# usnistgov/object-detection-yolov3

Measured on AMD Instinct MI355X. Metric: images/sec (train fwd+bwd) bs=8 416x416, higher is better.
Workload: dtype f32

## Files before the change

include/yolo3hip.h:

```cpp
#ifndef YOLO3HIP_H
#define YOLO3HIP_H

#include <math.h>
#include <stddef.h>
#include <stdint.h>

#ifdef __cplusplus
extern "C" {
#endif

#define Y3_OK 0
#define Y3_EINVAL (-1)
#define Y3_ELAUNCH (-2)

typedef void* y3_stream_t;

const char* y3_last_error(void);
int y3_debug_div(int x, int d);
int y3_version(void);

#define Y3_EPI_LRELU 1u
#define Y3_EPI_ACCUM 2u
#define Y3_CONV_X3 4u
int y3_x3_split_weights(const float* w, void* planes, int taps, int rows, int k_per_row, y3_stream_t stream);
int y3_x3_split_weights_batched(const float* arena, void* planes_arena, const int* table_dev, int nlayers, int total_blocks, y3_stream_t stream);
int y3_x3_prepare_weights_batched(const float* params, float* params_t, void* planes, void* planes_t, const int* table_dev, int nlayers,
                                  int total_tiles, y3_stream_t stream);

typedef struct y3_tensor {
    float* ptr;
    int n, h, w, c;
    int ld;
} y3_tensor;

int y3_conv2d_fwd(const y3_tensor* src, const float* wt, const float* bias, int ksize, int stride,
                  const y3_tensor* dst, unsigned flags, float alpha,
                  const float* scale, const float* shift, const y3_tensor* resid,
                  float* stats, void* workspace, size_t workspace_bytes, y3_stream_t stream);
int y3_conv2d_stats_tiles(int m, int cin, int ksize, int cout);
size_t y3_conv2d_fwd_workspace(int m, int cin, int ksize, int cout);
int y3_conv2d_stats_tiles_x(int m, int cin, int ksize, int cout, unsigned flags);
size_t y3_conv2d_fwd_workspace_x(int m, int cin, int ksize, int cout, unsigned flags);
int y3_conv2d_x3_ok(int m, int c, int ntaps, int nout);
int y3_conv2d_dgrad_x3_ok(const y3_tensor* ddst, int ksize, int stride, const y3_tensor* dsrc);
size_t y3_conv2d_plan(int m, int cin, int ksize, int cout, int* out13);
size_t y3_conv2d_plan_x(int m, int cin, int ksize, int cout, unsigned flags, int* out13);

int y3_conv2d_dgrad(const y3_tensor* ddst, const float* wt_t, int ksize, int stride,
                    const y3_tensor* dsrc, unsigned flags, void* workspace, size_t workspace_bytes,
                    y3_stream_t stream);
size_t y3_conv2d_dgrad_workspace(const y3_tensor* ddst, int ksize, int stride, const y3_tensor* dsrc);
size_t y3_conv2d_dgrad_workspace_x(const y3_tensor* ddst, int ksize, int stride, const y3_tensor* dsrc, unsigned flags);
int y3_conv2d_dgrad_bn(const y3_tensor* ddst, const float* wt_t, int ksize, int stride, const y3_tensor* dsrc,
                       unsigned flags, const y3_tensor* bn_a, float* bn_partials,
                       void* workspace, size_t workspace_bytes, y3_stream_t stream);
int y3_conv2d_dgrad_bn_tiles(const y3_tensor* ddst, int ksize, int stride, const y3_tensor* dsrc);
int y3_conv2d_dgrad_bn_tiles_x(const y3_tensor* ddst, int ksize, int stride, const y3_tensor* dsrc, unsigned flags);
size_t y3_conv2d_dgrad_plan_x(const y3_tensor* ddst, int ksize, int stride, const y3_tensor* dsrc, unsigned flags, int* out51);

int y3_conv2d_wgrad(const y3_tensor* src, const y3_tensor* ddst, int ksize, int stride,
                    float* dw, void* workspace, size_t workspace_bytes, y3_stream_t stream);
size_t y3_conv2d_wgrad_workspace(const y3_tensor* src, const y3_tensor* ddst, int ksize, int stride);
int y3_conv2d_wgrad_x(const y3_tensor* src, const y3_tensor* ddst, int ksize, int stride,
                      float* dw, unsigned flags, void* workspace, size_t workspace_bytes, y3_stream_t stream);
size_t y3_conv2d_wgrad_workspace_x(const y3_tensor* src, const y3_tensor* ddst, int ksize, int stride, unsigned flags);
int y3_conv2d_wgrad_x3_ok(int m, int cin, int ksize, int cout);
size_t y3_conv2d_wgrad_plan(int m, int cin, int ksize, int cout, int* out8);
size_t y3_conv2d_wgrad_plan_x(int m, int cin, int ksize, int cout, unsigned flags, int* out8);

int y3_transpose_weights(const float* wt, float* wt_t, int taps, int cin, int cout, y3_stream_t stream);
int y3_transpose_weights_batched(const float* params, float* params_t, const int* table_dev, int nlayers,
                                 int total_tiles, y3_stream_t stream);

int y3_bn_stats_finalize(const float* stats, int tiles, int c, int count,
                         const float* gamma, const float* beta, float eps, float momentum,
                         float* moving_mean, float* moving_var,
                         float* save_mean, float* save_rstd, float* scale, float* shift,
                         y3_stream_t stream);
int y3_bn_fold_inference(const float* gamma, const float* beta, const float* moving_mean,
                         const float* moving_var, float eps, int c, float* scale, float* shift,
                         y3_stream_t stream);
int y3_bn_fold_inference_batched(const float* params, const float* moving, float* chan, const int* table_dev,
                                 int nlayers, float eps, y3_stream_t stream);
int y3_bn_apply(const y3_tensor* a, const float* scale, const float* shift, const y3_tensor* resid,
                const y3_tensor* y, y3_stream_t stream);
int y3_bn_bwd_stats(const y3_tensor* dy, const y3_tensor* a, const y3_tensor* dres, int dres_accumulate,
                    const float* gamma, const float* save_mean, const float* save_rstd, float alpha,
                    float* dgamma, float* dbeta, float* dbias, float* coef,
                    void* workspace, size_t workspace_bytes, y3_stream_t stream);
size_t y3_bn_bwd_workspace(int m, int c);
int y3_bn_bwd_apply(const y3_tensor* dy, const y3_tensor* a, const float* coef, float alpha,
                    const y3_tensor* dz, y3_stream_t stream);
int y3_bn_bwd_apply_fanin(const y3_tensor* dy, const y3_tensor* a, const float* coef, float alpha,
                          const y3_tensor* dz, const y3_tensor* dres, int dres_accumulate, y3_stream_t stream);
int y3_bn_bwd_finalize_tiles(const float* partials, int tiles, int c, int count, const float* gamma,
                             const float* save_mean, const float* save_rstd, float alpha,
                             float* dgamma, float* dbeta, float* dbias, float* coef, y3_stream_t stream);
int y3_bn_frozen_bwd(const y3_tensor* dy, const y3_tensor* a, const y3_tensor* dres, int dres_accumulate,
                     const float* scale, const float* moving_mean, const float* moving_var, float eps, float alpha,
                     const y3_tensor* dz, float* dgamma, float* dbeta, float* dbias,
                     void* workspace, size_t workspace_bytes, y3_stream_t stream);
size_t y3_bn_frozen_bwd_workspace(int m, int c);

int y3_upsample_sum2x_fwd(const y3_tensor* in, const y3_tensor* out, y3_stream_t stream);
int y3_upsample_sum2x_bwd(const y3_tensor* dout, const y3_tensor* din, y3_stream_t stream);

#define Y3_SPP_MAX_PLANE 4096
int y3_spp_fwd(const y3_tensor* src, const y3_tensor* dst, y3_stream_t stream);
int y3_spp_fwd_bf16(const y3_tensor* src, const y3_tensor* dst, y3_stream_t stream);
int y3_spp_bwd(const y3_tensor* src, const y3_tensor* ddst, const y3_tensor* dsrc, int accumulate, y3_stream_t stream);

#define Y3_BF16_NO_PATCH 8u
int y3_conv2d_fwd_bf16(const y3_tensor* src, const void* wt_t_bf16, const float* bias, int ksize, int stride,
                       const y3_tensor* dst, int dst_is_f32, unsigned flags, float alpha,
                       const float* scale, const float* shift, const y3_tensor* resid, y3_stream_t stream);
size_t y3_conv2d_fwd_bf16_workspace(int m, int cin, int ksize, int cout);
int y3_conv2d_fwd_bf16_ws(const y3_tensor* src, const void* wt_t_bf16, const float* bias, int ksize, int stride,
                          const y3_tensor* dst, int dst_is_f32, unsigned flags, float alpha,
                          const float* scale, const float* shift, const y3_tensor* resid,
                          void* workspace, size_t workspace_bytes, y3_stream_t stream);
#define Y3_BF16_ROUTE_PP 1
#define Y3_BF16_ROUTE_C32 2
#define Y3_BF16_ROUTE_C64 3
#define Y3_BF16_ROUTE_RING 4
size_t y3_conv2d_fwd_bf16_plan(const y3_tensor* src, const void* wt_t_bf16, const float* bias, int ksize, int stride,
                               const y3_tensor* dst, int dst_is_f32, unsigned flags, float alpha,
// ... 269 lines not shown
```

object-detection-yolov3_amd/csrc/conv.hip:

```cpp
#include <stdlib.h>

#include <type_traits>
#include <utility>

#include "common.h"
#include "conv_plan.h"

template <int BM, int BN, int WM, int WN, int BK>
__global__ __launch_bounds__(64 * WM * WN) void conv_igemm_kernel(const ConvArgs p) {
    constexpr int THREADS = 64 * WM * WN;
    constexpr int LDA = BK + 4;
    constexpr int TM = BM / WM, TN = BN / WN, MB = TM / 32, NB = TN / 32;
    constexpr int KV = BK / 4;
    constexpr int A_TOTAL = BM * KV, A_LOADS = (A_TOTAL + THREADS - 1) / THREADS;
    constexpr int BN4 = BN / 4;
    constexpr int B_TOTAL = BK * BN4, B_LOADS = (B_TOTAL + THREADS - 1) / THREADS;
    static_assert(THREADS % KV == 0 && TM % 32 == 0 && TN % 32 == 0, "tile shape");

    __shared__ __attribute__((aligned(16))) float As[2][BM * LDA];
    __shared__ __attribute__((aligned(16))) float Bs[2][BK * BN];
    __shared__ float red[2][WM][BN];

    const int tid = threadIdx.x, lane = tid & 63, wave = tid >> 6;
    const int l31 = lane & 31, lh = lane >> 5;
// ... 893 lines not shown
    p.bn_part = a.bn_part;
    p.bn_a_ld = a.bn_a_ld;
    p.bn_a_bytes = a.bn_a ? (unsigned)((a.dense_dst ? (long long)a.M : (long long)a.src_n * a.DH * a.DW) * a.bn_a_ld * 4) : 0u;
    p.bn_row0 = 0;
    p.H = a.H;
    p.W = a.W;
    p.logC = a.logC;
    p.cmask = a.cmask;
    p.src_ld = a.src_ld;
    p.OH = a.OH;
    p.OW = a.OW;
    p.sh = a.sh;
    p.sw = a.sw;
    p.DH = a.DH;
    p.DW = a.DW;
    p.dsh = a.dsh;
    p.dsw = a.dsw;
    p.doh = a.doh;
    p.dow = a.dow;
    p.dst_ld = a.dst_ld;
    p.resid_ld = a.resid_ld;
    p.Nout = a.Nout;
    p.K = a.K;
    p.M = a.M;
    p.flags = a.flags;
    p.alpha = a.alpha;
    *f = p;
    return true;
}
static void set_split(FastArgs& f, const ConvPlan& pl) {
    f.dv_s0 = y3_make_div(pl.s0);
    f.dv_s1 = y3_make_div(pl.s1);
    f.sk_f = pl.f;
    f.sk_s0 = pl.s0;
    f.sk_s1 = pl.s1;
    f.sk_n0 = pl.f * pl.s0;
    f.sk_chunk0 = pl.chunk0;
    f.sk_chunk1 = pl.chunk1;
}

static int launch_igemm(const ConvArgs& a, const GemmDesc& d, void* workspace, size_t workspace_bytes, hipStream_t st) {
    ConvArgs p = a;
    const int ntaps = p.K / p.C;
    if (p.x3 && !d.x3) {
        y3_set_error("conv: Y3_CONV_X3 does not take this shape (C %d, Nout %d, K %d): ask y3_conv2d_x3_ok() first", p.C, p.Nout, p.K);
        return Y3_EINVAL;
    }
    ConvPlan pl = d.pl;
    if (no_room(pl.ws_bytes, workspace, workspace_bytes)) whole_tiles(pl, even_steps(p.K / pl.t.bk));
    const TileCfg t = pl.t;
    p.nbn = y3_cdiv(p.Nout, t.bn);
    FastArgs f;
    if (d.fast && make_fast(p, ntaps, t.bk, &f)) {
        f.nbn = p.nbn;
        f.nbm = y3_cdiv(p.M, t.bm);
        f.col_major = ((long long)p.K * p.Nout * 4 > 2048LL * 1024) ? 1 : 0;
        f.nb_fast = f.col_major ? f.nbm : f.nbn;
        f.dv_nb = y3_make_div(f.nb_fast);
        set_split(f, pl);
        f.sk_slab0 = pl.s0 > 1 ? 0 : f.sk_n0;
        f.tickets = pl.ws_bytes ? (int*)workspace : nullptr;
        if (f.tickets)
            if (int e = check_tickets("conv2d", workspace, st)) return e;
        f.slab = pl.ws_bytes ? (float*)((char*)workspace + Y3_WS_HEADER) : nullptr;
        const int grid = f.sk_n0 + (pl.tiles - pl.f) * pl.s1;
        const bool dense = p.dense_dst != 0;
        if (t.bk != 16) {
            y3_set_error("conv: the fast kernel is built for K steps of 16 (tile %dx%dx%d)", t.bm, t.bn, t.bk);
            return Y3_EINVAL;
        }
        if (p.bn_a && !dense) {
            y3_set_error("conv: BatchNorm-backward statistics need the dense fast kernel with K steps of 16");
            return Y3_EINVAL;
        }
        if (d.x3) {
            if (pl.short_last && pl.f == pl.tiles) f.x3_mode |= 8;
            if (!y3_x3_launch(f, t.bm, t.bn, dense, grid, st)) {
                y3_set_error("conv: no x3 kernel for tile %dx%d", t.bm, t.bn);
                return Y3_EINVAL;
            }
            Y3_CHECK_LAUNCH("conv_x3");
            return Y3_OK;
        }
        if (!launch_fast(t, f, dense, grid, st)) {
            y3_set_error("conv: no fast kernel for tile %dx%dx%d", t.bm, t.bn, t.bk);
            return Y3_EINVAL;
        }
        Y3_CHECK_LAUNCH("conv_igemm_fast");
        return Y3_OK;
    }
    if (p.bn_a || d.x3) {
        y3_set_error("conv: %s not available on the generic kernel (shape %d x %d x %d)", d.x3 ? "Y3_CONV_X3 is" : "BatchNorm-backward statistics are", p.M, p.Nout, p.K);
        return Y3_EINVAL;
    }
    if (!launch_generic(t, p, pl.tiles, st)) {
        y3_set_error("conv: no kernel for tile %dx%dx%d", t.bm, t.bn, t.bk);
        return Y3_EINVAL;
    }
    Y3_CHECK_LAUNCH("conv_igemm");
    return Y3_OK;
}

extern "C" int y3_conv2d_fwd(const y3_tensor* src, const float* wt, const float* bias, int ksize, int stride, const y3_tensor* dst,
                             unsigned flags, float alpha, const float* scale, const float* shift, const y3_tensor* resid, float* stats,
                             void* workspace, size_t workspace_bytes, y3_stream_t stream) {
    if (int e = check_tensor(src, "conv2d_fwd src")) return e;
    if (int e = check_tensor(dst, "conv2d_fwd dst")) return e;
    Y3_CHECK_ARG(wt, "conv2d_fwd: null weights");
    Y3_CHECK_ARG(ksize == 1 || ksize == 3, "conv2d_fwd: ksize %d unsupported", ksize);
    Y3_CHECK_ARG(stride == 1 || stride == 2, "conv2d_fwd: stride %d unsupported", stride);
    Y3_CHECK_ARG((src->c & 3) == 0, "conv2d_fwd: Cin=%d must be a multiple of 4", src->c);
    const int OH = (src->h + stride - 1) / stride, OW = (src->w + stride - 1) / stride;
    Y3_CHECK_ARG(dst->n == src->n && dst->h == OH && dst->w == OW, "conv2d_fwd: dst geometry %dx%dx%d != expected %dx%dx%d", dst->n,
                 dst->h, dst->w, src->n, OH, OW);
    Y3_CHECK_ARG((scale == nullptr) == (shift == nullptr), "conv2d_fwd: scale/shift must both be given");
    ConvArgs p = {};
    p.src = src->ptr;
    p.wt = wt;
    p.dst = dst->ptr;
    p.bias = bias;
    p.scale = scale;
    p.shift = shift;
    p.stats = stats;
    if (resid) {
        if (int e = check_tensor(resid, "conv2d_fwd resid")) return e;
        Y3_CHECK_ARG(resid->n == dst->n && resid->h == dst->h && resid->w == dst->w && resid->c == dst->c, "conv2d_fwd: resid geometry");
        p.resid = resid->ptr;
        p.resid_ld = resid->ld;
    }
    const int taps = ksize * ksize;
    if (int e = set_channels(src->c, taps, &p.logC, &p.cmask)) return e;
    const int pbh = y3_same_pad_before(src->h, ksize, stride), pbw = y3_same_pad_before(src->w, ksize, stride);
    for (int kh = 0; kh < ksize; ++kh)
        for (int kw = 0; kw < ksize; ++kw) {
            const int t = kh * ksize + kw;
            const int dh = kh - pbh, dw = kw - pbw;
            Y3_CHECK_ARG(dh >= -1 && dh <= 2 && dw >= -1 && dw <= 2, "conv2d_fwd: tap offset out of range");
            p.tap_dhdw |= (unsigned long long)((dh + 1) | ((dw + 1) << 2)) << (4 * t);
            p.tap_wsel |= (unsigned long long)t << (4 * t);
        }
    p.H = src->h;
    p.W = src->w;
    p.C = src->c;
    p.src_ld = src->ld;
    p.OH = OH;
    p.OW = OW;
    p.sh = p.sw = stride;
    p.DH = OH;
    p.DW = OW;
    p.dsh = p.dsw = 1;
    p.dst_ld = dst->ld;
    p.dense_dst = 1;
    p.Nout = dst->c;
    p.K = taps * src->c;
    p.M = src->n * OH * OW;
    p.flags = flags & ~Y3_CONV_X3;
    p.x3 = (flags & Y3_CONV_X3) ? 1 : 0;
    p.alpha = alpha;
    p.src_n = src->n;
    p.wt_rows = taps * src->c;
    return launch_igemm(p, describe_gemm(p), workspace, workspace_bytes, (hipStream_t)stream);
}

static int launch_dgrad_multi(const ConvArgs* cls, int ncls, MultiPlan pl, void* workspace, size_t workspace_bytes, hipStream_t st) {
    if (no_room(pl.ws, workspace, workspace_bytes)) {
        for (int c = 0; c < ncls; ++c) whole_tiles(pl.c[c], even_steps(cls[c].K / 16));
// ... 204 lines not shown
```

object-detection-yolov3_amd/csrc/conv_fast.h:

```cpp
#pragma once
#include <type_traits>
#include <utility>

#include "common.h"
#include "conv_plan.h"

struct FastArgs {
    const float* src;
    const float* wt;
    int Cper;
    int x3_mode;
    int korder;
    Y3Div dv_taps;
    float* dst;
    const float* bias;
    const float* scale;
    const float* shift;
    const float* resid;
    float* stats;
    int tap_off[9];
    int tap_wrow[9];
    int tg_nx, tg_off0, tg_offy, tg_offx, tg_w0, tg_wy, tg_wx;
    int tg_mul;
    int tap_dh[9], tap_dw[9];
    unsigned src_bytes, wt_bytes, dst_bytes, resid_bytes;
    int ntaps;
    int H, W, logC, cmask, src_ld;
    int OH, OW, sh, sw;
    int DH, DW, dsh, dsw, doh, dow, dst_ld;
    int resid_ld;
    int Nout, K, M;
    unsigned flags;
    float alpha;
    int nbn, nbm, col_major;
    int nb_fast, ohw;
    Y3Div dv_nb, dv_s0, dv_s1, dv_ohw, dv_ow;
    int sk_f, sk_n0, sk_s0, sk_s1, sk_chunk0, sk_chunk1;
    int sk_slab0;
    float* slab;
    int* tickets;
    const float* bn_a;
    float* bn_part;
    unsigned bn_a_bytes;
    int bn_a_ld;
    int bn_row0;
};

#define Y3_OOB 0x80000000u

#ifdef Y3_TIMING
__device__ int y3_abl_dev = 0;
#define Y3_ABL_INIT() const int y3_abl = __builtin_amdgcn_readfirstlane(y3_abl_dev)
#define Y3_ABL(bit) (y3_abl & (bit))
__device__ unsigned long long* y3_timing_buf = nullptr;
#define Y3_TSTAMP(i)                                                                                                    \
    do {                                                                                                                \
        if (y3_timing_buf && threadIdx.x == 0) y3_timing_buf[(size_t)blockIdx.x * 8 + (i)] = __builtin_amdgcn_s_memtime(); \
    } while (0)
#else
#define Y3_TSTAMP(i)
#define Y3_ABL_INIT()
#define Y3_ABL(bit) 0
#endif

template <int... I, class F>
__device__ __forceinline__ void y3_for_each_ic(std::integer_sequence<int, I...>, F&& f) {
    (f(std::integral_constant<int, I>{}), ...);
}
template <int MASK, int N>
__device__ __forceinline__ void y3_sgb() {
    if constexpr (N > 0) __builtin_amdgcn_sched_group_barrier(MASK, N, 0);
}
template <int COUNT, int MASK, int MFMAS = 1>
__device__ __forceinline__ void y3_sgb_pairs() {
    if constexpr (COUNT > 0) {
        y3_sgb<0x008, MFMAS>();
        y3_sgb<MASK, 1>();
        y3_sgb_pairs<COUNT - 1, MASK, MFMAS>();
    }
}

struct WgradArgs {
    const float* src;
    const float* ddst;
    float* out;
    unsigned long long tap_dhdw;
    int H, W, C, logC, cmask, src_ld;
    int OH, OW, sh, sw;
    int dd_ld, Nout, K, M;
    int chunk;
    int nbn, tiles, splits;
    unsigned src_bytes, dd_bytes;
    int* tickets;
    float* dw;
    int ohw, ntaps;
    Y3Div dv_tiles, dv_nbn, dv_ohw, dv_ow;
};

bool y3_wgrad_x3_launch(const WgradArgs& p, int bkr, int bn, unsigned grid, hipStream_t st);

bool y3_x3_launch(const FastArgs& p, int bm, int bn, bool dense, int grid, hipStream_t st);
struct FastArgs4 {
    FastArgs a[4];
    int first[5];
};
bool y3_x3_multi_launch(const FastArgs4& m, int bn, bool bns, int grid, hipStream_t st);
bool y3_x3_tile_ok(int bm, int bn);

struct FastWork {
    int tid, lane, wave, l31, lh, wm, wn;
    int bid0, bid, kz, nz;
    int bm, bn, m0, n0, kbeg, kend;
    int ohw, OW, aK, aM, aH, aW, src_ld, csh, csw, ntaps, Nout;
    Y3Div dv_ohw, dv_ow;
};

template <int BM, int BN, int WM, int WN, int BK, bool KZMAJOR = false, bool SHORTLAST = false>
__device__ __forceinline__ FastWork conv_fast_decode(const FastArgs& p, const int braw, const int grid) {
    FastWork w;
    const int tid = threadIdx.x, lane = tid & 63, wave = tid >> 6;
    const int l31 = lane & 31, lh = lane >> 5;
    const int wm = wave / WN, wn = wave % WN;
    int sk_n0 = p.sk_n0, sk_s0 = p.sk_s0, sk_s1 = p.sk_s1, sk_f = p.sk_f, sk_c0 = p.sk_chunk0, sk_c1 = p.sk_chunk1;
    int col_major = p.col_major, nb_fast = p.nb_fast, ohw = p.ohw, OW = p.OW, aK = p.K, aM = p.M, aH = p.H, aW = p.W;
    int src_ld = p.src_ld, csh = p.sh, csw = p.sw, ntaps = p.ntaps, Nout = p.Nout;
    unsigned dnb_m = p.dv_nb.mul, ds0_m = p.dv_s0.mul, ds1_m = p.dv_s1.mul, dohw_m = p.dv_ohw.mul, dow_m = p.dv_ow.mul;
    int dnb_s = p.dv_nb.shift, ds0_s = p.dv_s0.shift, ds1_s = p.dv_s1.shift, dohw_s = p.dv_ohw.shift, dow_s = p.dv_ow.shift;
    Y3_PIN_S(sk_n0); Y3_PIN_S(sk_s0); Y3_PIN_S(sk_s1); Y3_PIN_S(sk_f); Y3_PIN_S(sk_c0); Y3_PIN_S(sk_c1);
    Y3_PIN_S(col_major); Y3_PIN_S(nb_fast); Y3_PIN_S(ohw); Y3_PIN_S(OW); Y3_PIN_S(aK); Y3_PIN_S(aM); Y3_PIN_S(aH); Y3_PIN_S(aW);
    Y3_PIN_S(src_ld); Y3_PIN_S(csh); Y3_PIN_S(csw); Y3_PIN_S(ntaps); Y3_PIN_S(Nout);
    Y3_PIN_S(dnb_m); Y3_PIN_S(ds0_m); Y3_PIN_S(ds1_m); Y3_PIN_S(dohw_m); Y3_PIN_S(dow_m);
    Y3_PIN_S(dnb_s); Y3_PIN_S(ds0_s); Y3_PIN_S(ds1_s); Y3_PIN_S(dohw_s); Y3_PIN_S(dow_s);
    const Y3Div dv_nb = {dnb_m, dnb_s}, dv_s0 = {ds0_m, ds0_s}, dv_s1 = {ds1_m, ds1_s}, dv_ohw = {dohw_m, dohw_s}, dv_ow = {dow_m, dow_s};

    int bid0 = braw < sk_n0 ? y3_xcd_remap(braw, sk_n0) : sk_n0 + y3_xcd_remap(braw - sk_n0, grid - sk_n0);
    if (SHORTLAST && (p.x3_mode & 8) && sk_n0 == grid && sk_s0 > 1) {
        const int s = sk_s0, tiles = sk_f, nl = tiles * (s - 1);
        const int x = braw & 7, j = braw >> 3;
        const int ql = nl >> 3, rl = nl & 7;
        const int nlx = ql + (x < rl ? 1 : 0), l0 = x * ql + min(x, rl);
        if (j < nlx) {
            const int a = l0 + j, col = a / (nb_fast * (s - 1)), r = a - col * nb_fast * (s - 1), kzp = r / nb_fast;
            bid0 = (col * nb_fast + (r - kzp * nb_fast)) * s + kzp;
        } else {
            int s0x = 0;
            for (int y = 0; y < x; ++y) s0x += ((grid - y + 7) >> 3) - (ql + (y < rl ? 1 : 0));
            bid0 = (s0x + j - nlx) * s + (s - 1);
        }
    } else if (KZMAJOR && col_major) {
        const bool ra = bid0 < sk_n0;
        const int sl = ra ? sk_s0 : sk_s1;
        if (sl > 1) {
            const int t0 = ra ? 0 : sk_f, t1 = ra ? sk_f : sk_f + y3_div(grid - sk_n0, dv_s1);
            int a = ra ? bid0 : bid0 - sk_n0, base = t0;
            int n = min(t1, (y3_div(t0, dv_nb) + 1) * nb_fast) - t0;
            if (a >= n * sl) {
                a -= n * sl;
                base += n;
                const int col = a / (nb_fast * sl);
                a -= col * nb_fast * sl;
                base += col * nb_fast;
                n = min(nb_fast, t1 - base);
            }
            const int kzp = a / n;
            bid0 = (ra ? 0 : sk_n0) + (base + (a - kzp * n) - t0) * sl + kzp;
        }
    }
    int bid, kz, nz, kchunk;
    if (bid0 < sk_n0) {
        bid = y3_div(bid0, dv_s0);
        kz = bid0 - bid * sk_s0;
        nz = sk_s0;
        kchunk = sk_c0;
    } else {
        const int t = bid0 - sk_n0;
        const int q = y3_div(t, dv_s1);
        bid = sk_f + q;
        kz = t - q * sk_s1;
        nz = sk_s1;
        kchunk = sk_c1;
    }
    const int tq = y3_div(bid, dv_nb), tr = bid - tq * nb_fast;
    const int bm = col_major ? tr : tq;
    const int bn = col_major ? tq : tr;
    const int m0 = bm * BM, n0 = bn * BN;
    const int kbeg = kz * kchunk * BK;
    const int kend = min(aK, kbeg + kchunk * BK);
    w.tid = tid; w.lane = lane; w.wave = wave; w.l31 = l31; w.lh = lh; w.wm = wm; w.wn = wn;
    w.bid0 = bid0; w.bid = bid; w.kz = kz; w.nz = nz;
    w.bm = bm; w.bn = bn; w.m0 = m0; w.n0 = n0; w.kbeg = kbeg; w.kend = kend;
// ... 288 lines not shown
```

object-detection-yolov3_amd/csrc/conv_plan.cpp:

```cpp
#include <stdlib.h>
#include "host.h"
#include "conv_plan.h"

static TileCfg pick_tile(int M, int Nout) {
    TileCfg t;
    if (Nout <= 32)
        t = {128, 32, 16};
    else if (Nout <= 64)
        t = {128, 64, 16};
    else {
        const long long t128 = (long long)y3_cdiv(M, 128) * y3_cdiv(Nout, 128);
        const long long t64x128 = (long long)y3_cdiv(M, 64) * y3_cdiv(Nout, 128);
        if (t128 >= 600)
            t = {128, 128, 16};
        else if (t64x128 >= 600)
            t = {64, 128, 16};
        else
            t = {64, 64, 16};
    }
    return t;
}
void whole_tiles(ConvPlan& pl, int chunk) {
    pl.f = pl.tiles;
    pl.s0 = pl.s1 = 1;
// ... 49 lines not shown
            if (sc > 16) break;
            if ((long long)tiles * sc <= x3_slots)
                c_lo = c;
            else if (c_hi == 0 && (c_lo == 0 || sc > count_for(c_lo)))
                c_hi = c;
        }
        const int s_lo = c_lo > 0 ? count_for(c_lo) : 1;
        if (s_lo > 1) {
            pl.s0 = pl.s1 = s_lo;
            pl.chunk0 = pl.chunk1 = c_lo;
        }
        if (c_hi > 0 && ntaps == 9) {
            const int s_hi = count_for(c_hi), last = nk - (s_hi - 1) * c_hi;
            if ((long long)tiles * s_hi <= x3_slots + x3_slots / 16 && 3 * last <= c_hi) {
                pl.f = tiles;
                pl.s0 = pl.s1 = s_hi;
                pl.chunk0 = pl.chunk1 = c_hi;
                pl.short_last = 1;
                c_hi = 0;
            }
        }
        if (c_hi > 0) {
            const int s_hi = count_for(c_hi);
            const int f = (int)((x3_slots - (long long)tiles * s_lo) / (s_hi - s_lo));
            if (f > 0) {
                pl.f = f < tiles ? f : tiles;
                pl.s0 = s_hi;
                pl.chunk0 = c_hi;
            }
        }
    }
    pl.stats_tiles = y3_cdiv(M, pl.t.bm);
    size_slabs(pl, even_steps(nk));
    return pl;
}
static ConvPlan plan_conv(int M, int Nout, int K, bool fast_ok) {
    ConvPlan pl;
    pl.t = pick_tile(M, Nout);
    const int tiles = y3_cdiv(M, pl.t.bm) * y3_cdiv(Nout, pl.t.bn);
    const int nk = K / pl.t.bk;
    const int whole = nk > 0 ? nk : 1;
    pl.tiles = tiles;
    whole_tiles(pl, whole);
    constexpr int want = 2000;
    constexpr int min_k = 256;
    constexpr int cus = 256;
    constexpr int few_max = 512;
    const bool few_tiles = tiles <= few_max || ((long long)tiles * 2 <= want && K >= 2048);
    if (fast_ok && tiles <= Y3_MAX_TICKETS && few_tiles && K >= 2 * min_k) {
        int ks = (int)((want + tiles / 2) / tiles);
        const int maxs = K / min_k;
        if (ks > maxs) ks = maxs;
        if (ks > 16) ks = 16;
        if (ks > 1) {
            pl.chunk0 = even_steps(y3_cdiv(nk, ks));
            pl.s0 = y3_cdiv(nk, pl.chunk0);
        }
    } else if (fast_ok && tiles <= Y3_MAX_TICKETS && tiles > cus && nk >= 8) {
        const int F = tiles / cus * cus, R = tiles - F;
        if (R > 0) {
            int best = 1;
            double best_cost = 1.0;
            for (int S = 2; S <= 6 && S * 4 <= nk; ++S) {
                const double cost = (double)y3_cdiv((long long)R * S, cus) / S + 0.03 * (S - 1);
                if (cost < best_cost - 1e-9) {
                    best_cost = cost;
                    best = S;
                }
            }
            if (best > 1) {
                pl.f = F;
                pl.chunk1 = even_steps(y3_cdiv(nk, best));
                pl.s1 = y3_cdiv(nk, pl.chunk1);
            }
        }
    }
    pl.stats_tiles = y3_cdiv(M, pl.t.bm);
    size_slabs(pl, whole);
    return pl;
}
static bool fast_shape_ok(int C, int Nout, int K, int ntaps) {
    return !getenv("Y3_NO_FAST") && C % 16 == 0 && K % 16 == 0 && (ntaps == 1 || y3_is_pow2(C));
}
static GemmDesc describe_gemm(int M, int C, int ntaps, int Nout, unsigned flags) {
    GemmDesc d;
    const int K = ntaps * C;
    d.x3 = (flags & Y3_CONV_X3) && x3_shape_ok(C, Nout, K, ntaps);
    d.fast = d.x3 || fast_shape_ok(C, Nout, K, ntaps);
    d.pl = d.x3 ? plan_conv_x3(M, Nout, K, ntaps) : plan_conv(M, Nout, K, d.fast);
    return d;
}

extern "C" int y3_conv2d_x3_ok(int m, int c, int ntaps, int nout) {
    return (m > 0 && (ntaps == 1 || ntaps == 9 || ntaps == 2 || ntaps == 4) && x3_shape_ok(c, nout, ntaps * c, ntaps)) ? 1 : 0;
}
extern "C" int y3_conv2d_stats_tiles_x(int m, int cin, int ksize, int cout, unsigned flags) {
    return describe_gemm(m, cin, ksize * ksize, cout, flags).pl.stats_tiles;
}
extern "C" size_t y3_conv2d_fwd_workspace_x(int m, int cin, int ksize, int cout, unsigned flags) {
    return describe_gemm(m, cin, ksize * ksize, cout, flags).pl.ws_bytes;
}
extern "C" int y3_conv2d_stats_tiles(int m, int cin, int ksize, int cout) { return y3_conv2d_stats_tiles_x(m, cin, ksize, cout, 0u); }
extern "C" size_t y3_conv2d_fwd_workspace(int m, int cin, int ksize, int cout) { return y3_conv2d_fwd_workspace_x(m, cin, ksize, cout, 0u); }

extern "C" size_t y3_conv2d_plan(int m, int cin, int ksize, int cout, int* out13) { return y3_conv2d_plan_x(m, cin, ksize, cout, 0u, out13); }
extern "C" size_t y3_conv2d_plan_x(int m, int cin, int ksize, int cout, unsigned flags, int* out13) {
    const GemmDesc d = describe_gemm(m, cin, ksize * ksize, cout, flags);
    const ConvPlan& pl = d.pl;
    if (out13) {
        const int v[13] = {pl.t.bm, pl.t.bn, pl.t.bk, pl.tiles, pl.f, pl.s0, pl.s1, pl.chunk0, pl.chunk1,
                           pl.f * pl.s0 + (pl.tiles - pl.f) * pl.s1, pl.stats_tiles, (d.fast ? 1 : 0) | (pl.short_last ? 2 : 0), ksize * ksize * cin / pl.t.bk};
        for (int i = 0; i < 13; ++i) out13[i] = v[i];
    }
    return pl.ws_bytes;
}

bool fast_geom(const ConvArgs& a, int ntaps, int bk, FastGeom* g) {
    if (a.C % bk != 0 || a.K % bk != 0) return false;
    if (ntaps > 1 && !y3_is_pow2(a.C)) return false;
    g->min_off = 0;
    for (int t = 0; t < ntaps; ++t) {
        const int code = (int)((a.tap_dhdw >> (4 * t)) & 15ull);
        g->dh[t] = (code & 3) - 1;
        g->dw[t] = (code >> 2) - 1;
        const int off = (g->dh[t] * a.W + g->dw[t]) * a.src_ld;
        if (off < g->min_off) g->min_off = off;
    }
    const long long total = (long long)a.src_n * a.H * a.W * a.src_ld - g->min_off;
    const long long wtotal = (long long)(a.wt_rows) * a.Nout;
    if (total * 4 >= 0x7fffffffLL || wtotal * (a.x3 ? 6 : 4) >= 0x7fffffffLL) return false;
    g->src_bytes = (unsigned)(total * 4);
    g->wt_bytes = (unsigned)(wtotal * (a.x3 ? 6 : 4));
    for (int t = 0; t < ntaps; ++t) {
        g->off[t] = ((g->dh[t] * a.W + g->dw[t]) * a.src_ld - g->min_off) * 4;
        g->wrow[t] = (int)((a.tap_wsel >> (4 * t)) & 15ull) * a.C;
    }
    int nx = 1;
    while (nx < ntaps && g->dh[nx] == g->dh[0]) ++nx;
    if (ntaps % nx != 0 || nx > 3) return false;
    g->nx = nx;
    const int offx = nx > 1 ? g->off[1] - g->off[0] : 0, wx = nx > 1 ? g->wrow[1] - g->wrow[0] : 0;
    const int offy = ntaps > nx ? g->off[nx] - g->off[0] : 0, wy = ntaps > nx ? g->wrow[nx] - g->wrow[0] : 0;
    for (int t = 0; t < ntaps; ++t)
        if (g->off[t] != g->off[0] + (t / nx) * offy + (t % nx) * offx || g->wrow[t] != g->wrow[0] + (t / nx) * wy + (t % nx) * wx)
            return false;
    const long long dpix = a.dense_dst ? (long long)a.M : (long long)a.src_n * a.DH * a.DW;
    const long long db = dpix * a.dst_ld * 4, rb = dpix * (long long)a.resid_ld * 4;
    if (db >= 0x7fffffffLL || rb >= 0x7fffffffLL) return false;
    g->dst_bytes = (unsigned)db;
    g->resid_bytes = (unsigned)rb;
    return true;
}

GemmDesc describe_gemm(const ConvArgs& a) { return describe_gemm(a.M, a.C, a.K / a.C, a.Nout, a.x3 ? Y3_CONV_X3 : 0u); }

int set_channels(int C, int taps, int* logC, int* cmask) {
    if (taps == 1) {
        *logC = 31;
        *cmask = 0x7fffffff;
        return 0;
    }
    Y3_CHECK_ARG(y3_is_pow2(C) && C >= 4, "3x3 conv needs power-of-two channels >= 4 (got %d)", C);
    *logC = y3_ilog2(C);
    *cmask = C - 1;
    return 0;
}

static bool plan_dgrad_multi_f32(const ConvArgs* cls, int ncls, MultiPlan* pl) {
    int mmax = 0;
    for (int c = 0; c < ncls; ++c) mmax = cls[c].M > mmax ? cls[c].M : mmax;
    TileCfg t = pick_tile(mmax * ncls, cls[0].Nout);
    if (t.bm == 128 && t.bn == 128) t.bm = 64;
// ... 308 lines not shown
```

object-detection-yolov3_amd/csrc/conv_plan.h:

```cpp
#pragma once
#include "host.h"

struct ConvArgs {
    const float* src;
    const float* wt;
    float* dst;
    const float* bias;
    const float* scale;
    const float* shift;
    const float* resid;
    float* stats;
    unsigned long long tap_dhdw;
    unsigned long long tap_wsel;
    int H, W, C, logC, cmask, src_ld;
    int OH, OW, sh, sw;
    int DH, DW, dsh, dsw, doh, dow, dst_ld, dense_dst;
    int resid_ld;
    int Nout, K, M;
    unsigned flags;
    float alpha;
    int nbn;
    int src_n, wt_rows;
    const float* bn_a;
    float* bn_part;
    int bn_a_ld;
    int x3;
};

struct TileCfg {
    int bm, bn, bk;
};
#define Y3_WS_HEADER (256 * 1024)
#define Y3_MAX_TICKETS (Y3_WS_HEADER / 4)
static constexpr int x3_slots = 512;
struct ConvPlan {
    TileCfg t;
    int f, s0, s1, chunk0, chunk1;
    int tiles, stats_tiles;
    size_t ws_bytes;
    int short_last = 0;
};
static inline int even_steps(int chunk) { return chunk + (chunk & 1); }

struct GemmDesc {
    bool x3;
    bool fast;
    ConvPlan pl;
};

struct FastGeom {
    int min_off;
    int dh[9], dw[9], off[9], wrow[9];
    int nx;
    unsigned src_bytes, wt_bytes, dst_bytes, resid_bytes;
};

struct MultiPlan {
    ConvPlan c[4];
    int rows;
    size_t ws;
};

enum DgradHow {
    DGRAD_SINGLE,
    DGRAD_MERGED_F32,
    DGRAD_MERGED_X3,
    DGRAD_BY_CLASS
};
struct DgradDesc {
    ConvArgs cls[4];
    int ncls;
    DgradHow how;
    GemmDesc g[4];
    MultiPlan multi;
    int rows;
    size_t ws_bytes;
};

#define Y3_WG_FANIN 8
#define Y3_WG_TABLE 2048
struct WgradPlan {
    int bkr, bn, splits, chunk, tiles;
    bool x3;
    int grid;
    bool in_kernel;
    size_t ws_bytes;
};

void whole_tiles(ConvPlan& pl, int chunk);
bool no_room(size_t need, const void* workspace, size_t workspace_bytes);
bool fast_geom(const ConvArgs& a, int ntaps, int bk, FastGeom* g);
int set_channels(int C, int taps, int* logC, int* cmask);
GemmDesc describe_gemm(const ConvArgs& a);
bool dgrad_x3(unsigned flags, const y3_tensor* ddst, int ksize, int stride, const y3_tensor* dsrc);
int describe_dgrad(const y3_tensor* ddst, int ksize, int stride, const y3_tensor* dsrc, unsigned flags, DgradDesc* d);
WgradPlan describe_wgrad(int M, int cin, int taps, int Nout, unsigned flags);
```

object-detection-yolov3_amd/yolo3/_hip.py:

```python
import ctypes as C
import os

import torch

_HERE = os.path.dirname(os.path.abspath(__file__))
LIB_PATH = os.environ.get('Y3_LIB') or os.path.join(_HERE, '_lib', 'libyolo3hip.so')


class HipLibraryMissing(ImportError):
    pass


class HipError(RuntimeError):
    pass


if not os.path.exists(LIB_PATH):
    raise HipLibraryMissing(
        'libyolo3hip.so not found at %s: build it with `make -C object-detection-yolov3_amd/csrc` '
        '(hipcc --offload-arch=gfx950).  There is no CPU fallback.' % LIB_PATH)

lib = C.CDLL(LIB_PATH)


class Tensor(C.Structure):
    _fields_ = [('ptr', C.c_void_p), ('n', C.c_int), ('h', C.c_int), ('w', C.c_int), ('c', C.c_int), ('ld', C.c_int)]


class OptimDesc(C.Structure):
    _fields_ = [('kind', C.c_int), ('param', C.c_void_p), ('grad', C.c_void_p), ('m', C.c_void_p), ('v', C.c_void_p), ('count', C.c_size_t),
                ('hyper_dev', C.c_void_p), ('momentum', C.c_float), ('weight_decay', C.c_float), ('beta1', C.c_float), ('beta2', C.c_float),
                ('eps', C.c_float), ('decay_ranges_host', C.POINTER(C.c_longlong)), ('n_ranges', C.c_int), ('ema_param', C.c_void_p),
                ('moving', C.c_void_p), ('ema_moving', C.c_void_p), ('moving_count', C.c_size_t), ('omd_dev', C.c_void_p),
                ('scale_dev', C.c_void_p)]


TP = C.POINTER(Tensor)
vp, fp, ip = C.c_void_p, C.c_void_p, C.c_void_p
i32, u32, f32, sz = C.c_int, C.c_uint, C.c_float, C.c_size_t

SIGNATURES = {
    'y3_last_error': (C.c_char_p, []),
    'y3_debug_div': (i32, [i32, i32]),
    'y3_version': (i32, []),
    'y3_conv2d_fwd': (i32, [TP, fp, fp, i32, i32, TP, u32, f32, fp, fp, TP, fp, vp, sz, vp]),
    'y3_conv2d_stats_tiles': (i32, [i32, i32, i32, i32]),
    'y3_conv2d_fwd_workspace': (sz, [i32, i32, i32, i32]),
    'y3_conv2d_dgrad': (i32, [TP, fp, i32, i32, TP, u32, vp, sz, vp]),
    'y3_conv2d_stats_tiles_x': (i32, [i32, i32, i32, i32, u32]),
    'y3_conv2d_fwd_workspace_x': (sz, [i32, i32, i32, i32, u32]),
    'y3_conv2d_x3_ok': (i32, [i32, i32, i32, i32]),
    'y3_conv2d_dgrad_x3_ok': (i32, [TP, i32, i32, TP]),
    'y3_x3_split_weights': (i32, [fp, vp, i32, i32, i32, vp]),
    'y3_x3_split_weights_batched': (i32, [fp, vp, ip, i32, i32, vp]),
    'y3_x3_prepare_weights_batched': (i32, [fp, fp, vp, vp, ip, i32, i32, vp]),
    'y3_conv2d_dgrad_workspace_x': (sz, [TP, i32, i32, TP, u32]),
    'y3_conv2d_dgrad_bn_tiles_x': (i32, [TP, i32, i32, TP, u32]),
    'y3_conv2d_dgrad_workspace': (sz, [TP, i32, i32, TP]),
    'y3_conv2d_dgrad_bn': (i32, [TP, fp, i32, i32, TP, u32, TP, fp, vp, sz, vp]),
    'y3_conv2d_dgrad_bn_tiles': (i32, [TP, i32, i32, TP]),
    'y3_conv2d_wgrad': (i32, [TP, TP, i32, i32, fp, vp, sz, vp]),
    'y3_conv2d_wgrad_workspace': (sz, [TP, TP, i32, i32]),
    'y3_conv2d_wgrad_x': (i32, [TP, TP, i32, i32, fp, u32, vp, sz, vp]),
    'y3_conv2d_wgrad_workspace_x': (sz, [TP, TP, i32, i32, u32]),
    'y3_conv2d_wgrad_x3_ok': (i32, [i32, i32, i32, i32]),
    'y3_transpose_weights': (i32, [fp, fp, i32, i32, i32, vp]),
    'y3_transpose_weights_batched': (i32, [fp, fp, ip, i32, i32, vp]),
    'y3_bn_stats_finalize': (i32, [fp, i32, i32, i32, fp, fp, f32, f32, fp, fp, fp, fp, fp, fp, vp]),
    'y3_bn_fold_inference': (i32, [fp, fp, fp, fp, f32, i32, fp, fp, vp]),
    'y3_bn_fold_inference_batched': (i32, [fp, fp, fp, ip, i32, f32, vp]),
    'y3_bn_apply': (i32, [TP, fp, fp, TP, TP, vp]),
    'y3_bn_bwd_stats': (i32, [TP, TP, TP, i32, fp, fp, fp, f32, fp, fp, fp, fp, vp, sz, vp]),
    'y3_bn_bwd_workspace': (sz, [i32, i32]),
    'y3_bn_bwd_apply': (i32, [TP, TP, fp, f32, TP, vp]),
    'y3_bn_bwd_apply_fanin': (i32, [TP, TP, fp, f32, TP, TP, i32, vp]),
    'y3_bn_bwd_finalize_tiles': (i32, [fp, i32, i32, i32, fp, fp, fp, f32, fp, fp, fp, fp, vp]),
    'y3_bn_frozen_bwd': (i32, [TP, TP, TP, i32, fp, fp, fp, f32, f32, TP, fp, fp, fp, vp, sz, vp]),
    'y3_bn_frozen_bwd_workspace': (sz, [i32, i32]),
    'y3_upsample_sum2x_fwd': (i32, [TP, TP, vp]),
    'y3_upsample_sum2x_bwd': (i32, [TP, TP, vp]),
    'y3_spp_fwd': (i32, [TP, TP, vp]),
    'y3_spp_fwd_bf16': (i32, [TP, TP, vp]),
    'y3_spp_bwd': (i32, [TP, TP, TP, i32, vp]),
    'y3_copy': (i32, [TP, TP, vp]),
    'y3_conv2d_fwd_bf16': (i32, [TP, vp, fp, i32, i32, TP, i32, u32, f32, fp, fp, TP, vp]),
    'y3_conv2d_fwd_bf16_ws': (i32, [TP, vp, fp, i32, i32, TP, i32, u32, f32, fp, fp, TP, vp, sz, vp]),
    'y3_conv2d_fwd_bf16_workspace': (sz, [i32, i32, i32, i32]),
    'y3_conv2d_fwd_bf16_plan': (sz, [TP, vp, fp, i32, i32, TP, i32, u32, f32, fp, fp, TP, vp, sz, ip]),
    'y3_f32_to_bf16': (i32, [fp, vp, sz, vp]),
    'y3_conv2d_first_bf16': (i32, [TP, fp, fp, TP, u32, f32, fp, fp, vp]),
    'y3_tile_gather': (i32, [vp, i32, i32, i32, i32, ip, i32, i32, i32, fp, vp]),
    'y3_tile_gather_zscore_nhwc': (i32, [vp, i32, i32, i32, i32, ip, i32, i32, i32, fp, i32, vp, vp]),
    'y3_tile_gather_zscore_views_nhwc': (i32, [vp, i32, i32, i32, i32, ip, i32, i32, i32, C.POINTER(C.c_int), i32, fp, i32, vp, vp]),
    'y3_upsample_sum2x_fwd_bf16': (i32, [TP, TP, vp]),
    'y3_add_inplace': (i32, [TP, TP, vp]),
    'y3_fill': (i32, [fp, sz, f32, vp]),
    'y3_nchw_to_nhwc': (i32, [fp, i32, i32, i32, i32, TP, vp]),
    'y3_nhwc_to_nchw': (i32, [TP, fp, vp]),
    'y3_colsum': (i32, [TP, fp, vp]),
    'y3_decode_fwd': (i32, [TP, i32, C.POINTER(C.c_float), i32, i32, i32, i32, fp, vp]),
    'y3_loss_fwd_bwd': (i32, [TP, fp, C.POINTER(C.c_float), i32, i32, i32, i32, f32, fp, TP, vp, vp]),
    'y3_loss_fwd_bwd_ex': (i32, [TP, fp, C.POINTER(C.c_float), i32, i32, i32, i32, f32, i32, f32, fp, TP, vp, vp]),
    'y3_loss_workspace_bytes': (sz, []),
    'y3_truth_boxes': (i32, [fp, i32, C.c_longlong, i32, fp, ip, i32, vp]),
    'y3_loss_truth_workspace_bytes': (sz, [i32]),
    'y3_loss_fwd_bwd_truth': (i32, [TP, fp, C.POINTER(C.c_float), i32, i32, i32, i32, f32, i32, f32, fp, ip, i32, f32, fp, fp, TP, vp, vp]),
    'y3_loss_fwd_bwd_focal': (i32, [TP, fp, C.POINTER(C.c_float), i32, i32, i32, i32, f32, i32, f32, fp, ip, i32, f32, fp, fp, TP, vp, f32, f32, f32,
                                    f32, f32, vp]),
    'y3_adam_step': (i32, [fp, fp, fp, fp, sz, fp, f32, f32, f32, vp]),
    'y3_adam_step_ema': (i32, [fp, fp, fp, fp, sz, fp, f32, f32, f32, fp, fp, fp, sz, fp, vp]),
    'y3_grad_norm_workspace_bytes': (sz, [sz]),
    'y3_grad_accumulate': (i32, [fp, fp, sz, ip, vp, vp]),
    'y3_grad_sumsq': (i32, [fp, sz, vp, vp]),
    'y3_grad_clip_scale': (i32, [vp, sz, i32, C.c_double, fp, fp, vp]),
    'y3_adam_step_scaled': (i32, [fp, fp, fp, fp, sz, fp, f32, f32, f32, fp, vp]),
    'y3_adam_step_ema_scaled': (i32, [fp, fp, fp, fp, sz, fp, f32, f32, f32, fp, fp, fp, sz, fp, fp, vp]),
    'y3_optim_step': (i32, [C.POINTER(OptimDesc), vp]),
    'y3_nms_per_class': (i32, [fp, i32, i32, i32, f32, f32, f32, f32, f32, ip, ip, fp, i32, vp, sz, vp]),
    'y3_nms_workspace_bytes': (sz, [i32, i32, i32]),
    'y3_nms_single_class': (i32, [fp, i32, f32, ip, ip, fp, vp, sz, vp]),
    'y3_nms_per_class_ex': (i32, [fp, i32, i32, i32, i32, f32, f32, f32, f32, f32, f32, ip, ip, fp, i32, vp, sz, vp]),
    'y3_nms_workspace_bytes_ex': (sz, [i32, i32, i32, i32]),
    'y3_nms_labelled': (i32, [fp, i32, i32, i32, f32, f32, f32, ip, ip, fp, i32, vp, sz, vp]),
    'y3_tile_merge': (i32, [fp, i32, i32, i32, i32, ip, ip, fp, i32, ip, i32, i32, i32, i32, i32, f32, fp, i32, ip, vp, sz, vp]),
    'y3_tile_merge_workspace_bytes': (sz, [i32, i32]),
    'y3_tile_merge_voted': (i32, [fp, i32, i32, i32, ip, ip, i32, ip, i32, i32, i32, i32, i32, f32, fp, i32, ip, vp, sz, vp]),
    'y3_tta_views_nhwc': (i32, [fp, i32, i32, i32, i32, C.POINTER(C.c_int), i32, TP, vp]),
    'y3_tta_unmap': (i32, [fp, i32, i32, i32, C.POINTER(C.c_int), i32, i32, i32, vp]),
    'y3_box_vote': (i32, [fp, i32, i32, i32, ip, ip, fp, i32, f32, f32, f32, f32, f32, i32, i32, i32, fp, vp, sz, vp]),
    'y3_box_vote_workspace_bytes': (sz, [i32, i32, i32]),
    'y3_filter_small_boxes': (i32, [fp, i32, i32, f32, ip, ip, vp]),
    'y3_compute_iou': (i32, [fp, fp, i32, i32, fp, vp]),
    'y3_comm_unique_id': (i32, [vp]),
    'y3_comm_init': (i32, [vp, i32, i32, C.POINTER(C.c_void_p)]),
# ... 67 lines not shown
```

Measured before the change: 557.5.

## Add persistent row-streaming kernel for thin 1x1 convolutions with resident weights

```diff
diff --git a/include/yolo3hip.h b/include/yolo3hip.h
--- a/include/yolo3hip.h
+++ b/include/yolo3hip.h
@@ -42,6 +42,9 @@
 int y3_conv2d_stats_tiles_x(int m, int cin, int ksize, int cout, unsigned flags);
 size_t y3_conv2d_fwd_workspace_x(int m, int cin, int ksize, int cout, unsigned flags);
 int y3_conv2d_x3_ok(int m, int c, int ntaps, int nout);
+int y3_conv2d_stream_ok(int m, int k, int n, int taps);
+int y3_conv2d_stream_grid(int m, int k, int n, int taps);
+int y3_conv2d_stream_min_m(int min_m);
 int y3_conv2d_dgrad_x3_ok(const y3_tensor* ddst, int ksize, int stride, const y3_tensor* dsrc);
 size_t y3_conv2d_plan(int m, int cin, int ksize, int cout, int* out13);
 size_t y3_conv2d_plan_x(int m, int cin, int ksize, int cout, unsigned flags, int* out13);
diff --git a/object-detection-yolov3_amd/csrc/conv.hip b/object-detection-yolov3_amd/csrc/conv.hip
--- a/object-detection-yolov3_amd/csrc/conv.hip
+++ b/object-detection-yolov3_amd/csrc/conv.hip
@@ -999,6 +999,14 @@
             Y3_CHECK_LAUNCH("conv_x3");
             return Y3_OK;
         }
+        if (d.stream && dense && ntaps == 1 && p.sh == 1 && p.sw == 1 && p.H == p.OH && p.W == p.OW && f.tap_off[0] == 0 && !(p.bn_a && p.resid)) {
+            if (!y3_thin_launch(f, pl.tiles, thin_grid(pl.tiles), st)) {
+                y3_set_error("conv: no row-streaming kernel for K %d, Nout %d", p.K, p.Nout);
+                return Y3_EINVAL;
+            }
+            Y3_CHECK_LAUNCH("conv_thin");
+            return Y3_OK;
+        }
         if (!launch_fast(t, f, dense, grid, st)) {
             y3_set_error("conv: no fast kernel for tile %dx%dx%d", t.bm, t.bn, t.bk);
             return Y3_EINVAL;
diff --git a/object-detection-yolov3_amd/csrc/conv_fast.h b/object-detection-yolov3_amd/csrc/conv_fast.h
--- a/object-detection-yolov3_amd/csrc/conv_fast.h
+++ b/object-detection-yolov3_amd/csrc/conv_fast.h
@@ -106,6 +106,7 @@
 };
 bool y3_x3_multi_launch(const FastArgs4& m, int bn, bool bns, int grid, hipStream_t st);
 bool y3_x3_tile_ok(int bm, int bn);
+bool y3_thin_launch(const FastArgs& p, int ntiles, int grid, hipStream_t st);
 
 struct FastWork {
     int tid, lane, wave, l31, lh, wm, wn;
diff --git a/object-detection-yolov3_amd/csrc/conv_plan.cpp b/object-detection-yolov3_amd/csrc/conv_plan.cpp
--- a/object-detection-yolov3_amd/csrc/conv_plan.cpp
+++ b/object-detection-yolov3_amd/csrc/conv_plan.cpp
@@ -155,12 +155,36 @@
 static bool fast_shape_ok(int C, int Nout, int K, int ntaps) {
     return !getenv("Y3_NO_FAST") && C % 16 == 0 && K % 16 == 0 && (ntaps == 1 || y3_is_pow2(C));
 }
+static int thin_min_m = 0;
+static int thin_builtin_min_m(int K, int Nout) { return K == 128 ? 1024 * 128 : (Nout == 128 ? 600 * 128 : Y3_STREAM_MIN_M); }
+static bool thin_shape_ok(int K, int Nout, int ntaps) {
+    return ntaps == 1 && ((K == 64 && Nout == 32) || (K == 128 && Nout == 64) || (K == 32 && Nout == 64) || (K == 64 && Nout == 128));
+}
+extern "C" int y3_conv2d_stream_ok(int m, int k, int n, int taps) {
+    if (!thin_shape_ok(k, n, taps)) return 0;
+    if (thin_min_m > 0) return m >= thin_min_m ? 1 : 0;
+    if (m < thin_builtin_min_m(k, n)) return 0;
+    const ConvPlan pl = plan_conv(m, n, k, true);
+    return (pl.t.bm == 128 && pl.s0 == 1 && pl.s1 == 1) ? 1 : 0;
+}
+extern "C" int y3_conv2d_stream_grid(int m, int k, int n, int taps) { return y3_conv2d_stream_ok(m, k, n, taps) ? thin_grid(y3_cdiv(m, 128)) : 0; }
+extern "C" int y3_conv2d_stream_min_m(int min_m) {
+    const int old = thin_min_m;
+    if (min_m >= 0) thin_min_m = min_m;
+    return old;
+}
 static GemmDesc describe_gemm(int M, int C, int ntaps, int Nout, unsigned flags) {
     GemmDesc d;
     const int K = ntaps * C;
     d.x3 = (flags & Y3_CONV_X3) && x3_shape_ok(C, Nout, K, ntaps);
     d.fast = d.x3 || fast_shape_ok(C, Nout, K, ntaps);
     d.pl = d.x3 ? plan_conv_x3(M, Nout, K, ntaps) : plan_conv(M, Nout, K, d.fast);
+    d.stream = !d.x3 && d.fast && y3_conv2d_stream_ok(M, K, Nout, ntaps);
+    if (d.stream) {
+        d.pl.t = {128, Nout, 16};
+        d.pl.tiles = d.pl.stats_tiles = y3_cdiv(M, 128);
+        whole_tiles(d.pl, K / 16);
+    }
     return d;
 }
 
diff --git a/object-detection-yolov3_amd/csrc/conv_plan.h b/object-detection-yolov3_amd/csrc/conv_plan.h
--- a/object-detection-yolov3_amd/csrc/conv_plan.h
+++ b/object-detection-yolov3_amd/csrc/conv_plan.h
@@ -45,8 +45,12 @@
 struct GemmDesc {
     bool x3;
     bool fast;
+    bool stream;
     ConvPlan pl;
 };
+#define Y3_STREAM_MIN_M 43264
+static constexpr int thin_slots = 512;
+static inline int thin_grid(int tiles) { return tiles < thin_slots ? tiles : thin_slots; }
 
 struct FastGeom {
     int min_off;
diff --git a/object-detection-yolov3_amd/csrc/conv_thin.hip b/object-detection-yolov3_amd/csrc/conv_thin.hip
--- /dev/null
+++ b/object-detection-yolov3_amd/csrc/conv_thin.hip
@@ -0,0 +1,210 @@
+#include "common.h"
+#include "conv_fast.h"
+
+template <int BM, int BN, int WM, int WN>
+__device__ __forceinline__ void thin_finish_bns(const FastArgs& p, const int bm, const int tid, const int l31, const int lh, const int wm, const int wn,
+                                                f32x16 (&acc)[BM / WM / 32][BN / WN / 32], float (*red)[WM][BN]) {
+    constexpr int THREADS = 64 * WM * WN;
+    constexpr int TM = BM / WM, TN = BN / WN, MB = TM / 32, NB = TN / 32;
+    constexpr int G = MB * NB >= 4 ? 8 : 16;
+    const int m0 = bm * BM;
+    const bool do_lrelu = p.flags & Y3_EPI_LRELU;
+    const bool do_accum = p.flags & Y3_EPI_ACCUM;
+    float bsum[6][NB];
+#pragma unroll
+    for (int q = 0; q < 6; ++q)
+#pragma unroll
+        for (int j = 0; j < NB; ++j) bsum[q][j] = 0.f;
+    const __amdgpu_buffer_rsrc_t rs_dst = __builtin_amdgcn_make_buffer_rsrc(p.dst, 0, p.dst_bytes, 0x00020000);
+    const __amdgpu_buffer_rsrc_t rs_bna = __builtin_amdgcn_make_buffer_rsrc(const_cast<float*>(p.bn_a), 0, p.bn_a_bytes, 0x00020000);
+    const int mrow = m0 + wm * TM + 4 * lh;
+    const unsigned ld4 = (unsigned)p.dst_ld * 4u, ald4 = (unsigned)p.bn_a_ld * 4u;
+    const bool full = m0 + BM <= p.M;
+    const bool has_scale = p.scale != nullptr;
+#pragma unroll
+    for (int j = 0; j < NB; ++j) {
+        const int n = wn * TN + j * 32 + l31;
+        const bool nok = n < p.Nout;
+        const float bias = (p.bias && nok) ? p.bias[n] : 0.f;
+        const float sc = (has_scale && nok) ? p.scale[n] : 1.f;
+        const float sf = (has_scale && nok) ? p.shift[n] : 0.f;
+        const unsigned vbase = nok ? (unsigned)mrow * ld4 + (unsigned)n * 4u : Y3_OOB;
+        const unsigned abase = nok ? (unsigned)mrow * ald4 + (unsigned)n * 4u : Y3_OOB;
+#pragma unroll
+        for (int i = 0; i < MB; ++i) {
+#pragma unroll
+            for (int g = 0; g < 16 / G; ++g) {
+                float av[G], ex[G];
+#pragma unroll
+                for (int q = 0; q < G; ++q) {
+                    const int r = g * G + q, dr = i * 32 + (r & 3) + 8 * (r >> 2);
+                    const bool ok = full ? nok : (nok && mrow + dr < p.M);
+                    av[q] = __uint_as_float(__builtin_amdgcn_raw_buffer_load_b32(rs_bna, ok ? abase : Y3_OOB, (unsigned)dr * ald4, 0));
+                }
+                if (do_accum) {
+#pragma unroll
+                    for (int q = 0; q < G; ++q) {
+                        const int r = g * G + q, dr = i * 32 + (r & 3) + 8 * (r >> 2);
+                        const bool ok = full ? nok : (nok && mrow + dr < p.M);
+                        ex[q] = __uint_as_float(__builtin_amdgcn_raw_buffer_load_b32(rs_dst, ok ? vbase : Y3_OOB, (unsigned)dr * ld4, 0));
+                    }
+                }
+#pragma unroll
+                for (int q = 0; q < G; ++q) {
+                    const int r = g * G + q, dr = i * 32 + (r & 3) + 8 * (r >> 2);
+                    const bool ok = full ? nok : (nok && mrow + dr < p.M);
+                    float v = acc[i][j][r] + bias;
+                    if (do_lrelu) v = v > 0.f ? v : p.alpha * v;
+                    if (has_scale) v = v * sc + sf;
+                    if (do_accum) v += ex[q];
+                    const float dv = ok ? v : 0.f;
+                    const bool pos = av[q] > 0.f;
+                    bsum[0][j] += dv;
+                    bsum[1][j] += dv * av[q];
+                    bsum[2][j] += pos ? dv : 0.f;
+                    bsum[3][j] += pos ? av[q] : 0.f;
+                    bsum[4][j] += pos ? 1.f : 0.f;
+                    bsum[5][j] += av[q];
+                    __builtin_amdgcn_raw_buffer_store_b32(__float_as_uint(v), rs_dst, ok ? vbase : Y3_OOB, (unsigned)dr * ld4, 0);
+                }
+            }
+        }
+    }
+    y3_lds_barrier();
+#pragma unroll
+    for (int q = 0; q < 6; ++q)
+#pragma unroll
+        for (int j = 0; j < NB; ++j) {
+            const float s = bsum[q][j] + __shfl_xor(bsum[q][j], 32);
+            if (lh == 0) red[q][wm][wn * TN + j * 32 + l31] = s;
+        }
+    y3_lds_barrier();
+    for (int c = tid; c < 6 * BN; c += THREADS) {
+        const int which = c / BN, col = c % BN;
+        float s = 0.f;
+#pragma unroll
+        for (int w = 0; w < WM; ++w) s += red[which][w][col];
+        if (col < p.Nout) p.bn_part[((long long)(p.bn_row0 + bm) * 6 + which) * p.Nout + col] = s;
+    }
+}
+
+template <int KT, int BN, int WM, int WN, bool BNS>
+__global__ __launch_bounds__(256, 2) void conv_thin_kernel(const FastArgs p, const int ntiles) {
+    constexpr int BM = 128, BK = 16, THREADS = 256, LDA = BK + 4, KS = KT / BK;
+    constexpr int TM = BM / WM, TN = BN / WN, MB = TM / 32, NB = TN / 32;
+    constexpr int A_LOADS = BM * (BK / 4) / THREADS;
+    constexpr int W_LOADS = KT * BN / 4 / THREADS;
+    static_assert(WM * WN == 4 && KT % 32 == 0 && A_LOADS == 2 && (KT * BN / 4) % THREADS == 0, "tile shape");
+    static_assert(!BNS || 6 * WM * BN <= 2 * BM * LDA, "BNS column sums do not fit the A stage");
+
+    __shared__ __attribute__((aligned(16))) float As[2][BM * LDA];
+    __shared__ __attribute__((aligned(16))) float Ws[KT * BN];
+    __shared__ float red_own[BNS ? 1 : 2][BNS ? 1 : WM][BNS ? 1 : BN];
+    float (*red)[WM][BN] = BNS ? reinterpret_cast<float (*)[WM][BN]>(&As[0][0]) : reinterpret_cast<float (*)[WM][BN]>(&red_own[0][0][0]);
+
+    const int tid = threadIdx.x, lane = tid & 63, wave = tid >> 6;
+    const int l31 = lane & 31, lh = lane >> 5;
+    const int wm = wave / WN, wn = wave % WN;
+    const int grid = (int)gridDim.x;
+    const int aM = p.M, src_ld = p.src_ld;
+
+    const __amdgpu_buffer_rsrc_t rs_src = __builtin_amdgcn_make_buffer_rsrc(const_cast<float*>(p.src), 0, p.src_bytes, 0x00020000);
+    const __amdgpu_buffer_rsrc_t rs_wt = __builtin_amdgcn_make_buffer_rsrc(const_cast<float*>(p.wt), 0, p.wt_bytes, 0x00020000);
+
+    const int a_kv = tid & 3, a_row = tid >> 2;
+    unsigned a_voff[A_LOADS];
+#pragma unroll
+    for (int i = 0; i < A_LOADS; ++i) a_voff[i] = (unsigned)((a_row + i * (THREADS / 4)) * src_ld + a_kv * 4) * 4u;
+    const unsigned tile_bytes = (unsigned)(BM * src_ld) * 4u;
+
+    f32x4 ra[KS][A_LOADS];
+    auto gload = [&](int t, auto KSI) {
+        constexpr int ks = decltype(KSI)::value;
+        const unsigned soff = (t < ntiles ? (unsigned)t * tile_bytes : 0u) + (unsigned)p.tap_off[0] + (unsigned)(ks * BK * 4);
+#pragma unroll
+        for (int i = 0; i < A_LOADS; ++i) {
+            const bool ok = t * BM + a_row + i * (THREADS / 4) < aM;
+            ra[ks][i] = __builtin_amdgcn_raw_buffer_load_b128(rs_src, ok ? a_voff[i] : Y3_OOB, soff, 0);
+        }
+    };
+
+    int t = (int)blockIdx.x;
+    {
+        f32x4 rw[W_LOADS];
+#pragma unroll
+        for (int i = 0; i < W_LOADS; ++i) rw[i] = __builtin_amdgcn_raw_buffer_load_b128(rs_wt, (unsigned)(tid + i * THREADS) * 16u, 0, 0);
+        y3_for_each_ic(std::make_integer_sequence<int, KS>{}, [&](auto KSI) { gload(t, KSI); });
+#pragma unroll
+        for (int i = 0; i < W_LOADS; ++i) *reinterpret_cast<f32x4*>(&Ws[(tid + i * THREADS) * 4]) = rw[i];
+    }
+
+    const float* as_base = &As[0][(wm * TM + l31) * LDA + lh * 4];
+    const float* ws_base = &Ws[(lh * 4) * BN + wn * TN + l31];
+
+    for (; t < ntiles; t += grid) {
+        f32x16 acc[MB][NB];
+#pragma unroll
+        for (int i = 0; i < MB; ++i)
+#pragma unroll
+            for (int j = 0; j < NB; ++j)
+#pragma unroll
+                for (int r = 0; r < 16; ++r) acc[i][j][r] = 0.f;
+
+        y3_for_each_ic(std::make_integer_sequence<int, KS>{}, [&](auto KSI) {
+            constexpr int ks = decltype(KSI)::value, buf = ks & 1;
+#pragma unroll
+            for (int i = 0; i < A_LOADS; ++i) *reinterpret_cast<f32x4*>(&As[buf][(a_row + i * (THREADS / 4)) * LDA + a_kv * 4]) = ra[ks][i];
+            gload(t + grid, KSI);
+            y3_lds_barrier();
+#pragma unroll
+            for (int g = 0; g < 2; ++g) {
+                f32x4 fa[MB];
+                float fb[NB][4];
+#pragma unroll
+                for (int i = 0; i < MB; ++i) fa[i] = *reinterpret_cast<const f32x4*>(as_base + buf * (BM * LDA) + i * 32 * LDA + g * 8);
+#pragma unroll
+                for (int j = 0; j < NB; ++j)
+#pragma unroll
+                    for (int q = 0; q < 4; ++q) fb[j][q] = ws_base[(ks * BK + g * 8 + q) * BN + j * 32];
+#pragma unroll
+                for (int q = 0; q < 4; ++q)
+#pragma unroll
+                    for (int i = 0; i < MB; ++i)
+#pragma unroll
+                        for (int j = 0; j < NB; ++j) acc[i][j] = __builtin_amdgcn_mfma_f32_32x32x2f32(fa[i][q], fb[j][q], acc[i][j], 0, 0, 0);
+            }
+        });
+
+        if constexpr (BNS) {
+            thin_finish_bns<BM, BN, WM, WN>(p, t, tid, l31, lh, wm, wn, acc, red);
+            y3_lds_barrier();
+            continue;
+        }
+        FastWork fw;
+        fw.tid = tid; fw.lane = lane; fw.wave = wave; fw.l31 = l31; fw.lh = lh; fw.wm = wm; fw.wn = wn;
+        fw.bid0 = t; fw.bid = t; fw.kz = 0; fw.nz = 1;
+        fw.bm = t; fw.bn = 0; fw.m0 = t * BM; fw.n0 = 0; fw.kbeg = 0; fw.kend = KT;
+        fw.ohw = p.ohw; fw.OW = p.OW; fw.aK = KT; fw.aM = aM; fw.aH = p.H; fw.aW = p.W; fw.src_ld = src_ld; fw.csh = 1; fw.csw = 1; fw.ntaps = 1; fw.Nout = BN;
+        fw.dv_ohw = p.dv_ohw; fw.dv_ow = p.dv_ow;
+        conv_fast_finish<BM, BN, WM, WN, true, BNS>(p, fw, acc, red);
+        y3_lds_barrier();
+    }
+}
+
+template <int KT, int BN, int WM, int WN>
+static void launch_thin_cfg(const FastArgs& p, int ntiles, int grid, hipStream_t st) {
+    if (p.bn_a)
+        hipLaunchKernelGGL((conv_thin_kernel<KT, BN, WM, WN, true>), dim3(grid), dim3(256), 0, st, p, ntiles);
+    else
+        hipLaunchKernelGGL((conv_thin_kernel<KT, BN, WM, WN, false>), dim3(grid), dim3(256), 0, st, p, ntiles);
+}
+
+bool y3_thin_launch(const FastArgs& p, int ntiles, int grid, hipStream_t st) {
+    switch (p.K * 1000 + p.Nout) {
+        case 64 * 1000 + 32: launch_thin_cfg<64, 32, 4, 1>(p, ntiles, grid, st); return true;
+        case 128 * 1000 + 64: launch_thin_cfg<128, 64, 4, 1>(p, ntiles, grid, st); return true;
+        case 32 * 1000 + 64: launch_thin_cfg<32, 64, 4, 1>(p, ntiles, grid, st); return true;
+        case 64 * 1000 + 128: launch_thin_cfg<64, 128, 2, 2>(p, ntiles, grid, st); return true;
+    }
+    return false;
+}
diff --git a/object-detection-yolov3_amd/yolo3/_hip.py b/object-detection-yolov3_amd/yolo3/_hip.py
--- a/object-detection-yolov3_amd/yolo3/_hip.py
+++ b/object-detection-yolov3_amd/yolo3/_hip.py
@@ -50,6 +50,9 @@
     'y3_conv2d_stats_tiles_x': (i32, [i32, i32, i32, i32, u32]),
     'y3_conv2d_fwd_workspace_x': (sz, [i32, i32, i32, i32, u32]),
     'y3_conv2d_x3_ok': (i32, [i32, i32, i32, i32]),
+    'y3_conv2d_stream_ok': (i32, [i32, i32, i32, i32]),
+    'y3_conv2d_stream_grid': (i32, [i32, i32, i32, i32]),
+    'y3_conv2d_stream_min_m': (i32, [i32]),
     'y3_conv2d_dgrad_x3_ok': (i32, [TP, i32, i32, TP]),
     'y3_x3_split_weights': (i32, [fp, vp, i32, i32, i32, vp]),
     'y3_x3_split_weights_batched': (i32, [fp, vp, ip, i32, i32, vp]),
```

Result: no change. 561.6 (median of 6 runs) (+0.7%).
